# qhy991/llama.cpp-quant-gemm

Measured on NVIDIA B200. Metric: q4_0_q8_1_decode_gemv_hbm_gbs, higher is better.
Workload: dtype u4 x s8 -> s32 (dp4a), fp32 fold

## Files before the change

### llama.cpp-quant-gemm_b200/csrc/gemv.cu

```cuda
#include <cstdlib>

#include "ptx.cuh"
#include "qgemm_common.cuh"

namespace qgemm {

constexpr int kGemvWarps = 8;
constexpr int kGemvThreads = (kGemvWarps + 1) * 32;
constexpr int kGemvMaxStages = 8;
constexpr int kGemvInflightTarget = 56 * 1024;
constexpr int kGemvSlotsOff = 128;
constexpr int kGemvAbarOff = kGemvSlotsOff + 2 * kGemvWarps * 8 * 4;
constexpr int kGemvActOff = (kGemvAbarOff + 8 + 127) / 128 * 128;
static_assert(2 * kGemvMaxStages * 8 <= kGemvSlotsOff, "ring barriers overlap the slots");
static_assert(kGemvAbarOff % 8 == 0 && kGemvAbarOff + 8 <= kGemvActOff, "abar must not overlap the bulk-copy destination");
constexpr int kGemvSmemBudget = 110 * 1024;
constexpr int kGemvCtasPerSm = 2;
constexpr int kGemvMaxGroup = 8;
constexpr int kGemvTileTarget = 24 * 1024;

template <int WT> struct Pair { static constexpr int words = Fmt<WT>::bytes / 2; };

template <int WT>
__device__ __forceinline__ void load_pair(const uint8_t* p, uint32_t (&x)[Pair<WT>::words]) {
    if constexpr (WT == QGEMM_TYPE_Q5_1) {
        const uint4* q = reinterpret_cast<const uint4*>(p);
#pragma unroll
        for (int i = 0; i < 3; i++) {
            const uint4 v = q[i];
            x[4 * i] = v.x; x[4 * i + 1] = v.y; x[4 * i + 2] = v.z; x[4 * i + 3] = v.w;
        }
    } else if constexpr (WT == QGEMM_TYPE_Q4_1) {
        const uint2* q = reinterpret_cast<const uint2*>(p);
#pragma unroll
        for (int i = 0; i < 5; i++) {
            const uint2 v = q[i];
            x[2 * i] = v.x; x[2 * i + 1] = v.y;
        }
    } else {
        const uint32_t* q = reinterpret_cast<const uint32_t*>(p);
#pragma unroll
        for (int i = 0; i < Pair<WT>::words; i++) x[i] = q[i];
    }
}

__device__ __forceinline__ void expand4(const uint32_t (&q)[4], uint32_t (&w)[8]) {
#pragma unroll
    for (int i = 0; i < 4; i++) {
        w[i] = q[i] & 0x0f0f0f0fu;
        w[i + 4] = q[i] & 0xf0f0f0f0u;
    }
}
template <int WT>
__device__ __forceinline__ int pair_sumi(const uint32_t (&w)[8], const int (&a)[8]) {
    if constexpr (Fmt<WT>::bits == 4) {
        int lo = 0, hi = 0;
#pragma unroll
        for (int i = 0; i < 4; i++) {
            lo = dp4a_us(w[i], a[i], lo);
            hi = dp4a_us(w[i + 4], a[i + 4], hi);
        }
        return lo + (hi >> 4);
    } else {
        return block_sumi<WT>(w, a);
    }
}
__device__ __forceinline__ void expand5(const uint32_t (&q)[4], uint32_t qh, uint32_t (&w)[8]) {
#pragma unroll
    for (int i = 0; i < 4; i++) {
        w[i] = (q[i] & 0x0f0f0f0fu) | spread_qh4(qh, 4 * i);
        w[i + 4] = ((q[i] >> 4) & 0x0f0f0f0fu) | spread_qh4(qh, 16 + 4 * i);
    }
}

template <int WT>
__device__ __forceinline__ void expand_pair(const uint32_t (&x)[Pair<WT>::words], uint32_t (&w)[2][8], WScale (&ws)[2]) {
    auto fs = [](uint32_t lo, uint32_t hi) { return __funnelshift_r(lo, hi, 16); };
    if constexpr (WT == QGEMM_TYPE_Q4_0) {
        ws[0] = {half_bits_to_float(x[0]), 0.f};
        ws[1] = {half_bits_to_float(x[4] >> 16), 0.f};
        const uint32_t q0[4] = {fs(x[0], x[1]), fs(x[1], x[2]), fs(x[2], x[3]), fs(x[3], x[4])};
        const uint32_t q1[4] = {x[5], x[6], x[7], x[8]};
        expand4(q0, w[0]);
        expand4(q1, w[1]);
    } else if constexpr (WT == QGEMM_TYPE_Q4_1) {
        ws[0] = {half_bits_to_float(x[0]), half_bits_to_float(x[0] >> 16)};
        ws[1] = {half_bits_to_float(x[5]), half_bits_to_float(x[5] >> 16)};
        const uint32_t q0[4] = {x[1], x[2], x[3], x[4]};
        const uint32_t q1[4] = {x[6], x[7], x[8], x[9]};
        expand4(q0, w[0]);
        expand4(q1, w[1]);
    } else if constexpr (WT == QGEMM_TYPE_Q5_0) {
        ws[0] = {half_bits_to_float(x[0]), 0.f};
        ws[1] = {half_bits_to_float(x[5] >> 16), 0.f};
        const uint32_t q0[4] = {fs(x[1], x[2]), fs(x[2], x[3]), fs(x[3], x[4]), fs(x[4], x[5])};
        const uint32_t q1[4] = {x[7], x[8], x[9], x[10]};
        expand5(q0, fs(x[0], x[1]), w[0]);
        expand5(q1, x[6], w[1]);
    } else if constexpr (WT == QGEMM_TYPE_Q5_1) {
        ws[0] = {half_bits_to_float(x[0]), half_bits_to_float(x[0] >> 16)};
        ws[1] = {half_bits_to_float(x[6]), half_bits_to_float(x[6] >> 16)};
        const uint32_t q0[4] = {x[2], x[3], x[4], x[5]};
        const uint32_t q1[4] = {x[8], x[9], x[10], x[11]};
        expand5(q0, x[1], w[0]);
        expand5(q1, x[7], w[1]);
    } else {
        ws[0] = {half_bits_to_float(x[0]), 0.f};
        ws[1] = {half_bits_to_float(x[8] >> 16), 0.f};
#pragma unroll
        for (int i = 0; i < 8; i++) {
            w[0][i] = fs(x[i], x[i + 1]);
            w[1][i] = x[9 + i];
        }
    }
}

struct ActPair {
    int q[2][8];
    ActScale s[2];
};

struct GemvParams {
    const uint8_t* act;
    const uint8_t* wgt;
    float* C;
    int F, nb;
    int64_t ldc_t, ldc_f;
    int RT;
    int WPR;
    int stages;
    int stage_bytes;
    int pdl;
    int nocompute;
    int act_bulk;
    PeerOut peer;
    const uint8_t* pf_ptr;
    unsigned long long pf_bytes;
    int nmat;
    const uint8_t* wgt_m[kGemvMaxGroup];
    float* C_m[kGemvMaxGroup];
    int fstart[kGemvMaxGroup + 1];
    float skew;
#ifdef QGEMM_GEMV_TRACE
    int trace_slot;
#endif
};

#ifdef QGEMM_GEMV_TRACE
constexpr int kTraceSlots = 256, kTraceCtas = 304;
__device__ unsigned long long g_gemv_trace[kTraceSlots][kTraceCtas][6];
__device__ __forceinline__ unsigned long long gtimer() {
    unsigned long long t;
    asm volatile("mov.u64 %0, %%globaltimer;" : "=l"(t));
    return t;
}
#define GEMV_TRACE(i) do { if (threadIdx.x == 0 && blockIdx.x < kTraceCtas) g_gemv_trace[p.trace_slot][blockIdx.x][i] = gtimer(); } while (0)
#else
#define GEMV_TRACE(i)
#endif

struct TileRef { int m, local, rows; };
__device__ __forceinline__ TileRef tile_at(const GemvParams& p, int r0, int r_end) {
    TileRef t{0, r0, min(p.RT, r_end - r0)};
    if (p.nmat > 1) {
        int m = 0;
        while (m + 1 < p.nmat && r0 >= p.fstart[m + 1]) m++;
        t.m = m;
        t.local = r0 - p.fstart[m];
        t.rows = min(t.rows, p.fstart[m + 1] - r0);
    }
    return t;
}

template <int WT, int TT, int PPL, bool kMsExact, bool kFull>
__global__ void __launch_bounds__(kGemvThreads, kGemvCtasPerSm) gemv_kernel(const GemvParams p) {
    using Fm = Fmt<WT>;
    extern __shared__ __align__(128) uint8_t smem[];
    const int tid = threadIdx.x, warp = tid >> 5, lane = tid & 31;
    const int nb = p.nb, np = nb >> 1;

    uint64_t* full = reinterpret_cast<uint64_t*>(smem);
    uint64_t* empty = full + kGemvMaxStages;
    float* slots = reinterpret_cast<float*>(smem + kGemvSlotsOff);
    uint8_t* a_raw = smem + kGemvActOff;
    float4* a_scale = reinterpret_cast<float4*>(smem + kGemvActOff);
    uint4* a_qs = reinterpret_cast<uint4*>(smem + kGemvActOff + (size_t)TT * np * 16);
    const uint32_t act_bytes = (PPL > 0) ? (uint32_t)TT * nb * 36u : (uint32_t)TT * nb * 40u;
    uint8_t* stage0 = smem + (((uint32_t)kGemvActOff + act_bytes + 127u) & ~127u);

    auto span_at = [&](unsigned c) -> int {
        if (c >= gridDim.x) return p.F;
        const float x = (float)c / (float)gridDim.x;
        const float g = x * (1.0f + 0.5f * p.skew) - 0.5f * p.skew * x * x;
        return min(p.F, (int)((float)p.F * g + 0.5f));
    };
    const int r_begin = p.skew == 0.0f ? (int)(((int64_t)p.F * blockIdx.x) / gridDim.x) : span_at(blockIdx.x);
    const int r_end = p.skew == 0.0f ? (int)(((int64_t)p.F * (blockIdx.x + 1)) / gridDim.x) : span_at(blockIdx.x + 1);
    const size_t rowbytes = (size_t)nb * Fm::bytes;

    uint64_t* abar = reinterpret_cast<uint64_t*>(smem + kGemvAbarOff);
    if (tid == 0) {
        for (int s = 0; s < p.stages; s++) {
            ptx::mbar_init(&full[s], 1);
            ptx::mbar_init(&empty[s], kGemvWarps);
        }
        ptx::mbar_init(abar, 1);
        ptx::fence_mbar_init();
    }
    __syncthreads();
    if (p.pdl) ptx::griddep_launch_dependents();

    if (warp == kGemvWarps) {
        if (lane == 0) {
            int s = 0;
            uint32_t ph = 0;
            for (int r0 = r_begin; r0 < r_end;) {
                const TileRef tr = tile_at(p, r0, r_end);
                const uint8_t* src = (p.nmat > 1 ? p.wgt_m[tr.m] : p.wgt) + (size_t)tr.local * rowbytes;
                const uint32_t bytes = (uint32_t)(tr.rows * rowbytes);
                ptx::mbar_wait(&empty[s], ph ^ 1);
                ptx::mbar_arrive_expect_tx(&full[s], bytes);
                ptx::bulk_g2s(stage0 + (size_t)s * p.stage_bytes, src, bytes, &full[s]);
                if (++s == p.stages) { s = 0; ph ^= 1; }
                r0 += tr.rows;
            }
            if (p.pf_ptr) {
                const unsigned long long chunk = ((p.pf_bytes / gridDim.x) + 15ull) & ~15ull;
                unsigned long long off = chunk * blockIdx.x;
                const unsigned long long end = min(off + chunk, p.pf_bytes & ~15ull);
                for (; off < end; off += 16384ull)
                    ptx::bulk_prefetch_l2(p.pf_ptr + off, (uint32_t)min(16384ull, end - off));
            }
        }
        return;
    }

    GEMV_TRACE(0);
    if (p.pdl == 1) ptx::griddep_wait();
    GEMV_TRACE(1);
    if (p.peer.world > 1) {
        if (tid == 0) peer_wait_prior(p.peer);
        ptx::bar_sync(1, kGemvWarps * 32);
    }
    const int WPR = p.WPR;
    const int rpp = kGemvWarps / WPR;
    const int rslot = warp / WPR, sub = warp - rslot * WPR;

    ActPair areg[PPL > 0 ? TT : 1][PPL > 0 ? PPL : 1];
    if constexpr (PPL > 0) {
        const uint32_t* a32 = reinterpret_cast<const uint32_t*>(p.act);
        uint32_t* dst = reinterpret_cast<uint32_t*>(a_raw);
        const int total = TT * nb * 9;
        if (p.act_bulk) {
            if (tid == 0) {
                ptx::mbar_arrive_expect_tx(abar, (uint32_t)total * 4u);
                ptx::bulk_g2s(a_raw, p.act, (uint32_t)total * 4u, abar);
            }
            ptx::mbar_wait(abar, 0);
            GEMV_TRACE(4);
        } else {
            for (int i = tid; i < total; i += kGemvWarps * 32) dst[i] = __ldg(a32 + i);
            ptx::bar_sync(1, kGemvWarps * 32);
        }
#pragma unroll
        for (int j = 0; j < PPL; j++) {
            const int pg = (j * WPR + sub) * 32 + lane;
#pragma unroll
            for (int t = 0; t < TT; t++) {
                if (kFull || j < PPL - 1 || pg < np) {
                    const uint32_t* w = dst + ((size_t)t * nb + 2 * pg) * 9;
#pragma unroll
                    for (int b = 0; b < 2; b++) {
                        const uint32_t ds = w[9 * b];
                        areg[t][j].s[b] = prep_act_scale<WT, kMsExact>(half_bits_to_float(ds), half_bits_to_float(ds >> 16));
#pragma unroll
                        for (int i = 0; i < 8; i++) areg[t][j].q[b][i] = (int)w[9 * b + 1 + i];
                    }
                }
            }
        }
    } else {
        const uint32_t* a32 = reinterpret_cast<const uint32_t*>(p.act);
        float* sc = reinterpret_cast<float*>(a_scale);
        uint32_t* qs = reinterpret_cast<uint32_t*>(a_qs);
        const int total = TT * nb * 9;
        for (int i = tid; i < total; i += kGemvWarps * 32) {
            const int blk = i / 9, wd = i - blk * 9;
            const int t = blk / nb, b = blk - t * nb;
            const uint32_t v = __ldg(a32 + i);
            if (wd == 0) {
                const ActScale ps = prep_act_scale<WT, kMsExact>(half_bits_to_float(v), half_bits_to_float(v >> 16));
                float* d = sc + ((size_t)t * np + (b >> 1)) * 4 + (b & 1) * 2;
                d[0] = ps.d;
                d[1] = ps.s;
            } else {
                const int e = wd - 1;
                const int quad = (b & 1) * 2 + (e >> 2);
                qs[(((size_t)t * 4 + quad) * np + (b >> 1)) * 4 + (e & 3)] = v;
            }
        }
        ptx::bar_sync(1, kGemvWarps * 32);
    }

    GEMV_TRACE(2);
    int s = 0, spar = 0;
    uint32_t ph = 0;
    const int npl = (PPL > 0) ? PPL : (np + WPR * 32 - 1) / (WPR * 32);
    for (int g0 = r_begin; g0 < r_end;) {
        const TileRef tr = tile_at(p, g0, r_end);
        const int r0 = tr.local, rows = tr.rows;
        float* Cm = p.nmat > 1 ? p.C_m[tr.m] : p.C;
        g0 += rows;
        ptx::mbar_wait(&full[s], ph);
        const uint8_t* tile = stage0 + (size_t)s * p.stage_bytes;
        for (int pass = 0; pass * rpp < rows && !p.nocompute; pass++) {
            const int r = pass * rpp + rslot;
            float acc[TT];
#pragma unroll
            for (int tt = 0; tt < TT; tt++) acc[tt] = 0.f;
            if (r < rows) {
                const uint8_t* rowp = tile + (size_t)r * rowbytes;
                auto do_pair = [&](int j, int pg) {
                    uint32_t x[Pair<WT>::words];
                    uint32_t w[2][8];
                    WScale ws[2];
                    load_pair<WT>(rowp + (size_t)pg * (2 * Fm::bytes), x);
                    expand_pair<WT>(x, w, ws);
#pragma unroll
                    for (int tt = 0; tt < TT; tt++) {
                        if constexpr (PPL > 0) {
                            const ActPair& a = areg[tt][j];
                            acc[tt] = fold_block_pre<WT>(acc[tt], pair_sumi<WT>(w[0], a.q[0]), ws[0], a.s[0]);
                            acc[tt] = fold_block_pre<WT>(acc[tt], pair_sumi<WT>(w[1], a.q[1]), ws[1], a.s[1]);
                        } else {
                            const float4 sc = a_scale[(size_t)tt * np + pg];
                            int a0[8], a1[8];
                            const uint4 q0 = a_qs[((size_t)tt * 4 + 0) * np + pg];
                            const uint4 q1 = a_qs[((size_t)tt * 4 + 1) * np + pg];
                            const uint4 q2 = a_qs[((size_t)tt * 4 + 2) * np + pg];
                            const uint4 q3 = a_qs[((size_t)tt * 4 + 3) * np + pg];
                            a0[0] = q0.x; a0[1] = q0.y; a0[2] = q0.z; a0[3] = q0.w;
                            a0[4] = q1.x; a0[5] = q1.y; a0[6] = q1.z; a0[7] = q1.w;
                            a1[0] = q2.x; a1[1] = q2.y; a1[2] = q2.z; a1[3] = q2.w;
                            a1[4] = q3.x; a1[5] = q3.y; a1[6] = q3.z; a1[7] = q3.w;
                            acc[tt] = fold_block_pre<WT>(acc[tt], pair_sumi<WT>(w[0], a0), ws[0], ActScale{sc.x, sc.y});
                            acc[tt] = fold_block_pre<WT>(acc[tt], pair_sumi<WT>(w[1], a1), ws[1], ActScale{sc.z, sc.w});
                        }
                    }
                };
                if constexpr (PPL > 0) {
#pragma unroll
                    for (int j = 0; j < PPL; j++) {
                        const int pg = (j * WPR + sub) * 32 + lane;
                        if (kFull || j < PPL - 1 || pg < np) do_pair(j, pg);
                    }
                } else {
                    for (int j = 0; j < npl; j++) {
                        const int pg = (j * WPR + sub) * 32 + lane;
                        if (pg < np) do_pair(0, pg);
                    }
                }
            }
#pragma unroll
            for (int tt = 0; tt < TT; tt++) {
#pragma unroll
                for (int o = 16; o > 0; o >>= 1) acc[tt] += __shfl_xor_sync(0xffffffffu, acc[tt], o);
            }
            if (WPR == 1) {
                if (r < rows && lane < TT) {
                    float v = acc[0];
#pragma unroll
                    for (int tt = 1; tt < TT; tt++) v = (lane == tt) ? acc[tt] : v;
                    peer_store(p.peer, Cm, (int64_t)lane * p.ldc_t + (int64_t)(r0 + r) * p.ldc_f, v, tr.m);
                }
            } else {
                float* sl = slots + spar * (kGemvWarps * 8);
                if (lane == 0) {
#pragma unroll
                    for (int tt = 0; tt < TT; tt++) sl[warp * 8 + tt] = acc[tt];
                }
                ptx::bar_sync(2 + rslot, WPR * 32);
                if (sub == 0 && lane < TT && r < rows) {
                    float v = 0.f;
                    for (int k = 0; k < WPR; k++) v += sl[(rslot * WPR + k) * 8 + lane];
                    peer_store(p.peer, Cm, (int64_t)lane * p.ldc_t + (int64_t)(r0 + r) * p.ldc_f, v, tr.m);
                }
                spar ^= 1;
            }
        }
        __syncwarp();
        if (lane == 0) ptx::mbar_arrive(&empty[s]);
        if (++s == p.stages) { s = 0; ph ^= 1; }
    }
    GEMV_TRACE(3);
    if (p.peer.world > 1) {
        if (!(p.peer.dbg & 4)) __threadfence();
        ptx::bar_sync(1, kGemvWarps * 32);
        if (tid == 0) peer_signal_done(p.peer, gridDim.x);
    }
    if (p.pdl == 2) ptx::griddep_wait();
}

struct GemvPlan {
    int tt;
    int ppl;
    int wpr;
    int rt;
    int stages, stage_bytes;
    size_t smem;
};

static bool gemv_plan(int wtype, int T, int F, int K, int grid, bool pdl, GemvPlan* pl);

bool gemv_supported(int wtype, const void* act, const void* wgt, int F, int K) {
    const int nb = K / 32;
    const size_t rowbytes = (size_t)nb * block_bytes(wtype);
    if (F < 1 || nb < 2 || (nb & 1)) return false;
    if (rowbytes % 16 != 0 || rowbytes > 64 * 1024) return false;
    if (reinterpret_cast<uintptr_t>(wgt) % 16 != 0) return false;
    if (reinterpret_cast<uintptr_t>(act) % 4 != 0) return false;
    GemvPlan pl;
    return gemv_plan(wtype, 1, F, K, 1, false, &pl);
}

static bool gemv_plan(int wtype, int T, int F, int K, int grid, bool pdl, GemvPlan* pl) {
    const int nb = K / 32, np = nb / 2;
    const size_t rowbytes = (size_t)nb * block_bytes(wtype);
    for (int tt = min(T, 8); tt >= 1; tt--) {
        int ppl = 0, wpr = 1;
        for (int w = 1; w <= kGemvWarps; w <<= 1) {
            const int need = (np + 32 * w - 1) / (32 * w);
            if (need * tt <= 3) { ppl = need; wpr = w; break; }
        }
        if (QGEMM_ENV("QGEMM_GEMV_FORCE_SMEM")) ppl = 0;
        if (ppl == 0) {
            wpr = 1;
            while (wpr < kGemvWarps && np > 64 * wpr) wpr <<= 1;
        }
        const int rpp = kGemvWarps / wpr;
        int rt = rpp;
        while (rt < 8 && (size_t)(2 * rt) * rowbytes <= (size_t)kGemvTileTarget) rt <<= 1;
        if (const char* e = QGEMM_ENV("QGEMM_GEMV_RT")) rt = max(rpp, atoi(e) / rpp * rpp);
        const size_t fixed = kGemvActOff + (size_t)tt * nb * (ppl == 0 ? 40 : 36) + 128;
        auto stage_of = [&](int r) { return (int)(((size_t)r * rowbytes + 127) / 128 * 128); };
        while (rt > 1 && fixed + 2 * (size_t)stage_of(rt) > (size_t)kGemvSmemBudget) rt >>= 1;
        const int stage_bytes = stage_of(rt);
        if (fixed + 2 * (size_t)stage_bytes > (size_t)kGemvSmemBudget) continue;
        int stages = (int)(((size_t)kGemvSmemBudget - fixed) / stage_bytes);
        stages = max(2, min(kGemvMaxStages, stages));
        const int rows_per_cta = (F + grid - 1) / grid;
        stages = max(2, min(stages, (rows_per_cta + rt - 1) / rt));
        stages = max(2, min(stages, kGemvInflightTarget / stage_bytes));
        (void)pdl;
        if (const char* e = QGEMM_ENV("QGEMM_GEMV_STAGES")) stages = max(2, min(kGemvMaxStages, atoi(e)));
        *pl = {tt, ppl, wpr, rt, stages, stage_bytes, fixed + (size_t)stages * stage_bytes};
        return true;
    }
    return false;
}

template <int WT, int TT, int PPL>
static cudaError_t launch_gemv_inst(const GemvParams& p, size_t smem, int grid, bool ms_exact, cudaStream_t st) {
    auto launch = [&](auto kernel, int variant) -> cudaError_t {
        (void)variant;
        if (cudaError_t e = smem_optin(reinterpret_cast<const void*>(kernel), smem)) return e;
        cudaLaunchConfig_t cfg{};
        cfg.gridDim = dim3(grid);
        cfg.blockDim = dim3(kGemvThreads);
        cfg.dynamicSmemBytes = smem;
        cfg.stream = st;
        cudaLaunchAttribute at[1];
        at[0].id = cudaLaunchAttributeProgrammaticStreamSerialization;
        at[0].val.programmaticStreamSerializationAllowed = 1;
        cfg.attrs = at;
        cfg.numAttrs = p.pdl ? 1 : 0;
        return cudaLaunchKernelEx(&cfg, kernel, p);
    };
    cudaError_t e;
    const bool full = PPL > 0 && (p.nb / 2) == PPL * p.WPR * 32;
    if constexpr (Fmt<WT>::m >= 0) {
        if (full) e = ms_exact ? launch(gemv_kernel<WT, TT, PPL, true, true>, 2) : launch(gemv_kernel<WT, TT, PPL, false, true>, 3);
        else e = ms_exact ? launch(gemv_kernel<WT, TT, PPL, true, false>, 1) : launch(gemv_kernel<WT, TT, PPL, false, false>, 0);
    } else {
        e = full ? launch(gemv_kernel<WT, TT, PPL, false, true>, 3) : launch(gemv_kernel<WT, TT, PPL, false, false>, 0);
    }
    note_launch();
    return e;
}

template <int WT>
static cudaError_t launch_gemv_wt(const GemvPlan& pl, const GemvParams& p, int grid, bool ms, cudaStream_t st) {
#define QG_CASE(TTv, PPLv) \
    if (pl.tt == TTv && pl.ppl == PPLv) return launch_gemv_inst<WT, TTv, PPLv>(p, pl.smem, grid, ms, st);
    QG_CASE(1, 1) QG_CASE(1, 2) QG_CASE(1, 3) QG_CASE(2, 1) QG_CASE(3, 1)
    QG_CASE(1, 0) QG_CASE(2, 0) QG_CASE(3, 0) QG_CASE(4, 0) QG_CASE(5, 0) QG_CASE(6, 0) QG_CASE(7, 0) QG_CASE(8, 0)
#undef QG_CASE
    return cudaErrorInvalidValue;
}

struct GemvGroup { int nmat; const void* wgt[kGemvMaxGroup]; float* C[kGemvMaxGroup]; int F[kGemvMaxGroup]; };

cudaError_t launch_gemv(int wtype, const void* act, const void* wgt, float* C, int T, int F, int K, int64_t ldc_t,
                        int64_t ldc_f, uint32_t flags, int num_sms, cudaStream_t st, const PeerOut* peer,
                        const void* pf_ptr, size_t pf_bytes, const GemvGroup* group);

cudaError_t launch_gemv(int wtype, const void* act, const void* wgt, float* C, int T, int F, int K, int64_t ldc_t,
                        int64_t ldc_f, uint32_t flags, int num_sms, cudaStream_t st, const PeerOut* peer,
                        const void* pf_ptr, size_t pf_bytes) {
    return launch_gemv(wtype, act, wgt, C, T, F, K, ldc_t, ldc_f, flags, num_sms, st, peer, pf_ptr, pf_bytes, nullptr);
}

cudaError_t launch_gemv(int wtype, const void* act, const void* wgt, float* C, int T, int F, int K, int64_t ldc_t,
                        int64_t ldc_f, uint32_t flags, int num_sms, cudaStream_t st, const PeerOut* peer,
                        const void* pf_ptr, size_t pf_bytes, const GemvGroup* group) {
    const int nb = K / 32;
    const bool ms = flags & QGEMM_MS_EXACT;
    GemvPlan pl;
    int ctas_per_sm = kGemvCtasPerSm;
    if (const char* e = QGEMM_ENV("QGEMM_GEMV_CTAS")) ctas_per_sm = max(1, min(kGemvCtasPerSm, atoi(e)));
    const int grid = min(F, ctas_per_sm * num_sms);
    const bool pdl = flags & QGEMM_WEIGHTS_STATIC;
    if (!gemv_plan(wtype, T, F, K, grid, pdl, &pl)) return cudaErrorInvalidValue;
    for (int t0 = 0; t0 < T; t0 += pl.tt) {
        GemvPlan cur = pl;
        if (T - t0 < pl.tt && !gemv_plan(wtype, T - t0, F, K, grid, pdl, &cur)) return cudaErrorInvalidValue;
        GemvParams p;
        p.act = (const uint8_t*)act + (size_t)t0 * nb * kQ81Bytes;
        p.wgt = (const uint8_t*)wgt;
        p.C = C + (int64_t)t0 * ldc_t;
        p.F = F; p.nb = nb; p.ldc_t = ldc_t; p.ldc_f = ldc_f;
        p.RT = cur.rt; p.WPR = cur.wpr; p.stages = cur.stages; p.stage_bytes = cur.stage_bytes;
        p.pdl = pdl ? ((flags & QGEMM_INPUTS_READY) ? 2 : 1) : 0;
        p.nocompute = QGEMM_ENV("QGEMM_GEMV_NOCOMPUTE") ? 1 : 0;
        p.act_bulk = (reinterpret_cast<uintptr_t>(p.act) % 16 == 0 && ((size_t)cur.tt * nb * kQ81Bytes) % 16 == 0 &&
                      !QGEMM_ENV("QGEMM_GEMV_NO_ACT_BULK")) ? 1 : 0;
        p.pf_ptr = (t0 + pl.tt >= T && reinterpret_cast<uintptr_t>(pf_ptr) % 16 == 0) ? (const uint8_t*)pf_ptr : nullptr;
        p.pf_bytes = pf_bytes;
        p.skew = QGEMM_ENV("QGEMM_GEMV_SKEW") ? (float)atof(QGEMM_ENV("QGEMM_GEMV_SKEW")) : (F >= 8 * grid ? 0.28f : 0.0f);
#ifdef QGEMM_GEMV_TRACE
        {
            static int seq = 0;
            p.trace_slot = seq++ % kTraceSlots;
        }
#endif
        p.nmat = 0;
        if (group && group->nmat == 1) {
            p.wgt = (const uint8_t*)group->wgt[0];
            p.C = group->C[0] + (int64_t)t0 * ldc_t;
        } else if (group) {
            p.nmat = group->nmat;
            p.fstart[0] = 0;
            for (int m = 0; m < group->nmat; m++) {
                p.wgt_m[m] = (const uint8_t*)group->wgt[m];
                p.C_m[m] = group->C[m] + (int64_t)t0 * ldc_t;
                p.fstart[m + 1] = p.fstart[m] + group->F[m];
            }
        }
        p.peer = PeerOut{};
        if (peer) {
            if (T > pl.tt) return cudaErrorInvalidValue;
            p.peer = *peer;
        }
        cudaError_t e;
        switch (wtype) {
        case QGEMM_TYPE_Q4_0: e = launch_gemv_wt<QGEMM_TYPE_Q4_0>(cur, p, grid, ms, st); break;
        case QGEMM_TYPE_Q4_1: e = launch_gemv_wt<QGEMM_TYPE_Q4_1>(cur, p, grid, ms, st); break;
        case QGEMM_TYPE_Q5_0: e = launch_gemv_wt<QGEMM_TYPE_Q5_0>(cur, p, grid, ms, st); break;
        case QGEMM_TYPE_Q5_1: e = launch_gemv_wt<QGEMM_TYPE_Q5_1>(cur, p, grid, ms, st); break;
        case QGEMM_TYPE_Q8_0: e = launch_gemv_wt<QGEMM_TYPE_Q8_0>(cur, p, grid, ms, st); break;
        default: e = cudaErrorInvalidValue;
        }
        if (e != cudaSuccess) return e;
    }
    return cudaSuccess;
}


constexpr int kChainMaxSteps = 160;
constexpr int kChainMaxMat = 3;
constexpr int kChainQStride = 1536 * 36;

struct ChainStep {
    const uint8_t* act;
    const float* x;
    const float* gate;
    const uint8_t* wgt[kChainMaxMat];
    float* C[kChainMaxMat];
    int fstart[kChainMaxMat + 1];
    int nb;
    int ldc_f;
    unsigned char nmat, RT, WPR, ppl, full, wait;
};

template <int NS> struct ChainParams {
    int nsteps;
    int stages, stage_bytes;
    uint32_t act_bytes;
    unsigned* sync;
    uint8_t* qscratch;
    int pdl;
    const uint8_t* pf_ptr;
    unsigned long long pf_bytes;
    ChainStep st[NS];
};
constexpr int kChainSmall = 8;

__device__ __forceinline__ uint32_t ld_acquire_gpu(const unsigned* p) {
    uint32_t v;
    asm volatile("ld.acquire.gpu.global.u32 %0, [%1];" : "=r"(v) : "l"(p) : "memory");
    return v;
}

struct ChainTile { int m, local, rows; };
__device__ __forceinline__ ChainTile chain_tile_at(const ChainStep& st, int r0, int r_end) {
    int m = 0;
    while (m + 1 < st.nmat && r0 >= st.fstart[m + 1]) m++;
    return {m, r0 - st.fstart[m], min(min((int)st.RT, r_end - r0), st.fstart[m + 1] - r0)};
}

__device__ __forceinline__ int chain_round_half_away(float v) {
    const float t = truncf(v);
    const float r = v - t;
    int q = __float2int_rz(t);
    if (fabsf(r) >= 0.5f) q += (v < 0.0f) ? -1 : 1;
    return q;
}
__device__ __noinline__ void chain_quantize_block_lanes(const float* x, const float* gate, uint8_t* out, int lane) {
    float v = __ldcg(x + lane);
    if (gate) v = __fmul_rn(__fdiv_rn(v, __fadd_rn(1.0f, expf(-v))), __ldcg(gate + lane));
    float amax = fabsf(v);
#pragma unroll
    for (int o = 16; o > 0; o >>= 1) amax = fmaxf(amax, __shfl_xor_sync(0xffffffffu, amax, o));
    float sum = 0.0f;
#pragma unroll
    for (int j = 0; j < 32; j++) sum = __fadd_rn(sum, __shfl_sync(0xffffffffu, v, j));
    const float d = __fdiv_rn(amax, 127.0f);
    const float id = (d > 0.0f) ? __fdiv_rn(1.0f, d) : 0.0f;
    const int q = max(-128, min(127, chain_round_half_away(__fmul_rn(v, id))));
    out[4 + lane] = (uint8_t)(q & 0xff);
    if (lane == 0)
        *reinterpret_cast<uint32_t*>(out) =
            (uint32_t)__half_as_ushort(__float2half_rn(d)) | ((uint32_t)__half_as_ushort(__float2half_rn(sum)) << 16);
}

template <int WT, int PPL, bool kFull>
__device__ __forceinline__ void chain_consume(const ChainStep& st, const int r_begin, const int r_end, const uint32_t* araw,
                                              const uint8_t* stage0, const int stage_bytes, const int nstages, uint64_t* full,
                                              uint64_t* empty, float* slots, int& s, uint32_t& ph, int& spar) {
    using Fm = Fmt<WT>;
    const int tid = threadIdx.x, warp = tid >> 5, lane = tid & 31;
    const int nb = st.nb, np = nb >> 1;
    const int WPR = st.WPR;
    const int rpp = kGemvWarps / WPR;
    const int rslot = warp / WPR, sub = warp - rslot * WPR;
    const size_t rowbytes = (size_t)nb * Fm::bytes;

    ActPair areg[PPL];
#pragma unroll
    for (int j = 0; j < PPL; j++) {
        const int pg = (j * WPR + sub) * 32 + lane;
        if (kFull || j < PPL - 1 || pg < np) {
            const uint32_t* w = araw + (size_t)(2 * pg) * 9;
#pragma unroll
            for (int b = 0; b < 2; b++) {
                const uint32_t ds = w[9 * b];
                areg[j].s[b] = prep_act_scale<WT, false>(half_bits_to_float(ds), half_bits_to_float(ds >> 16));
#pragma unroll
                for (int i = 0; i < 8; i++) areg[j].q[b][i] = (int)w[9 * b + 1 + i];
            }
        }
    }
    for (int g0 = r_begin; g0 < r_end;) {
        const ChainTile tr = chain_tile_at(st, g0, r_end);
        const int r0 = tr.local, rows = tr.rows;
        float* Cm = st.C[tr.m];
        g0 += rows;
        ptx::mbar_wait(&full[s], ph);
        const uint8_t* tile = stage0 + (size_t)s * stage_bytes;
        for (int pass = 0; pass * rpp < rows; pass++) {
            const int r = pass * rpp + rslot;
            float acc = 0.f;
            if (r < rows) {
                const uint8_t* rowp = tile + (size_t)r * rowbytes;
#pragma unroll
                for (int j = 0; j < PPL; j++) {
                    const int pg = (j * WPR + sub) * 32 + lane;
                    if (kFull || j < PPL - 1 || pg < np) {
                        uint32_t x[Pair<WT>::words];
                        uint32_t w[2][8];
                        WScale ws[2];
                        load_pair<WT>(rowp + (size_t)pg * (2 * Fm::bytes), x);
                        expand_pair<WT>(x, w, ws);
                        acc = fold_block_pre<WT>(acc, pair_sumi<WT>(w[0], areg[j].q[0]), ws[0], areg[j].s[0]);
                        acc = fold_block_pre<WT>(acc, pair_sumi<WT>(w[1], areg[j].q[1]), ws[1], areg[j].s[1]);
                    }
                }
            }
#pragma unroll
            for (int o = 16; o > 0; o >>= 1) acc += __shfl_xor_sync(0xffffffffu, acc, o);
            if (WPR == 1) {
                if (r < rows && lane == 0) Cm[(int64_t)(r0 + r) * st.ldc_f] = acc;
            } else {
                float* sl = slots + spar * (kGemvWarps * 8);
                if (lane == 0) sl[warp * 8] = acc;
                ptx::bar_sync(2 + rslot, WPR * 32);
                if (sub == 0 && lane == 0 && r < rows) {
                    float v = 0.f;
                    for (int k = 0; k < WPR; k++) v += sl[(rslot * WPR + k) * 8];
                    Cm[(int64_t)(r0 + r) * st.ldc_f] = v;
                }
                spar ^= 1;
            }
        }
        __syncwarp();
        if (lane == 0) ptx::mbar_arrive(&empty[s]);
        if (++s == nstages) { s = 0; ph ^= 1; }
    }
}

template <int WT, int NS>
__global__ void __launch_bounds__(kGemvThreads, kGemvCtasPerSm) gemv_chain_kernel(const __grid_constant__ ChainParams<NS> p) {
    using Fm = Fmt<WT>;
    extern __shared__ __align__(128) uint8_t smem[];
    const int tid = threadIdx.x, warp = tid >> 5, lane = tid & 31;
    uint64_t* full = reinterpret_cast<uint64_t*>(smem);
    uint64_t* empty = full + kGemvMaxStages;
    float* slots = reinterpret_cast<float*>(smem + kGemvSlotsOff);
    uint64_t* abar = reinterpret_cast<uint64_t*>(smem + kGemvAbarOff);
    uint8_t* a_raw = smem + kGemvActOff;
    uint8_t* stage0 = smem + (((uint32_t)kGemvActOff + p.act_bytes + 127u) & ~127u);
    const unsigned grid = gridDim.x;

    if (tid == 0) {
        for (int s = 0; s < p.stages; s++) {
            ptx::mbar_init(&full[s], 1);
            ptx::mbar_init(&empty[s], kGemvWarps);
        }
        ptx::mbar_init(abar, 1);
        ptx::fence_mbar_init();
    }
    __syncthreads();
    if (p.pdl) ptx::griddep_launch_dependents();

    if (warp == kGemvWarps) {
        if (lane == 0) {
            int s = 0;
            uint32_t ph = 0;
            for (int k = 0; k < p.nsteps; k++) {
                const ChainStep& st = p.st[k];
                const int F = st.fstart[st.nmat];
                const int r_begin = (int)(((int64_t)F * blockIdx.x) / grid);
                const int r_end = (int)(((int64_t)F * (blockIdx.x + 1)) / grid);
                const size_t rowbytes = (size_t)st.nb * Fm::bytes;
                for (int r0 = r_begin; r0 < r_end;) {
                    const ChainTile tr = chain_tile_at(st, r0, r_end);
                    const uint8_t* src = st.wgt[tr.m] + (size_t)tr.local * rowbytes;
                    const uint32_t bytes = (uint32_t)(tr.rows * rowbytes);
                    ptx::mbar_wait(&empty[s], ph ^ 1);
                    ptx::mbar_arrive_expect_tx(&full[s], bytes);
                    ptx::bulk_g2s(stage0 + (size_t)s * p.stage_bytes, src, bytes, &full[s]);
                    if (++s == p.stages) { s = 0; ph ^= 1; }
                    r0 += tr.rows;
                }
            }
            if (p.pf_ptr) {
                const unsigned long long chunk = ((p.pf_bytes / grid) + 15ull) & ~15ull;
                unsigned long long off = chunk * blockIdx.x;
                const unsigned long long end = min(off + chunk, p.pf_bytes & ~15ull);
                for (; off < end; off += 16384ull)
                    ptx::bulk_prefetch_l2(p.pf_ptr + off, (uint32_t)min(16384ull, end - off));
            }
        }
        return;
    }

    if (p.pdl) ptx::griddep_wait();
    int s = 0, spar = 0;
    uint32_t ph = 0, aph = 0;
    for (int k = 0; k < p.nsteps; k++) {
        const ChainStep& st = p.st[k];
        const int F = st.fstart[st.nmat];
        const int r_begin = (int)(((int64_t)F * blockIdx.x) / grid);
        const int r_end = (int)(((int64_t)F * (blockIdx.x + 1)) / grid);
        if (st.act) {
            if (tid == 0) {
                if (st.wait && k > 0)
                    while (ld_acquire_gpu(p.sync + (k - 1)) < grid) __nanosleep(20);
                const uint32_t bytes = (uint32_t)st.nb * 36u;
                ptx::mbar_arrive_expect_tx(abar, bytes);
                ptx::bulk_g2s(a_raw, st.act, bytes, abar);
            }
            ptx::mbar_wait(abar, aph);
            aph ^= 1;
        } else {
            if (k > 0) {
                if (tid == 0)
                    while (ld_acquire_gpu(p.sync + (k - 1)) < grid) __nanosleep(20);
                ptx::bar_sync(1, kGemvWarps * 32);
            }
            uint8_t* qbuf = p.qscratch + (size_t)(k & 1) * kChainQStride;
            for (int b = (int)blockIdx.x + warp * (int)grid; b < st.nb; b += kGemvWarps * (int)grid)
                chain_quantize_block_lanes(st.x + (size_t)b * 32, st.gate ? st.gate + (size_t)b * 32 : nullptr, qbuf + (size_t)b * 36, lane);
            __threadfence();
            ptx::bar_sync(1, kGemvWarps * 32);
            if (tid == 0) {
                atomicAdd(p.sync + p.nsteps + 1 + k, 1u);
                while (ld_acquire_gpu(p.sync + p.nsteps + 1 + k) < grid) __nanosleep(20);
            }
            ptx::bar_sync(1, kGemvWarps * 32);
            const uint32_t* src = reinterpret_cast<const uint32_t*>(qbuf);
            uint32_t* dst = reinterpret_cast<uint32_t*>(a_raw);
            for (int i = tid; i < st.nb * 9; i += kGemvWarps * 32) dst[i] = __ldcg(src + i);
            ptx::fence_proxy_async();
            ptx::bar_sync(1, kGemvWarps * 32);
        }
        const uint32_t* araw = reinterpret_cast<const uint32_t*>(a_raw);
#define QG_CHAIN_CASE(P, FULL) \
    chain_consume<WT, P, FULL>(st, r_begin, r_end, araw, stage0, p.stage_bytes, p.stages, full, empty, slots, s, ph, spar)
        if (st.full) {
            if (st.ppl == 1) QG_CHAIN_CASE(1, true);
            else if (st.ppl == 2) QG_CHAIN_CASE(2, true);
            else QG_CHAIN_CASE(3, true);
        } else {
            if (st.ppl == 1) QG_CHAIN_CASE(1, false);
            else if (st.ppl == 2) QG_CHAIN_CASE(2, false);
            else QG_CHAIN_CASE(3, false);
        }
#undef QG_CHAIN_CASE
        if (lane == 0) __threadfence();
        ptx::bar_sync(1, kGemvWarps * 32);
        if (tid == 0) atomicAdd(p.sync + k, 1u);
    }
    if (tid == 0) {
        if (atomicAdd(p.sync + p.nsteps, 1u) == grid - 1) {
            for (int k = 0; k <= 2 * p.nsteps; k++) p.sync[k] = 0u;
        }
    }
}

struct ChainStepHost {
    const void* act; const float* x; const float* gate;
    int nmat; const void* wgt[kChainMaxMat]; float* C[kChainMaxMat]; int F[kChainMaxMat];
    int K; int ldc_f; int wait;
};

int gemv_chain_max_steps() { return kChainMaxSteps; }
static size_t gemv_chain_counter_bytes(int) { return ((size_t)(2 * kChainMaxSteps + 1) * sizeof(unsigned) + 255) / 256 * 256; }
size_t gemv_chain_sync_bytes(int nsteps) { return gemv_chain_counter_bytes(nsteps) + 2 * (size_t)kChainQStride; }

template <int NS>
static bool gemv_chain_plan(int wtype, const ChainStepHost* steps, int nsteps, int grid, ChainParams<NS>* out, size_t* smem) {
    if (nsteps < 1 || nsteps > NS) return false;
    int stage_bytes = 0;
    size_t act_bytes = 0;
    for (int k = 0; k < nsteps; k++) {
        const ChainStepHost& h = steps[k];
        if (h.nmat < 1 || h.nmat > kChainMaxMat) return false;
        const int nb = h.K / 32;
        int Ftot = 0;
        for (int m = 0; m < h.nmat; m++) {
            if (!gemv_supported(wtype, h.act ? h.act : (const void*)h.x, h.wgt[m], h.F[m], h.K)) return false;
            Ftot += h.F[m];
        }
        if (h.act) {
            if (reinterpret_cast<uintptr_t>(h.act) % 16 != 0 || ((size_t)nb * kQ81Bytes) % 16 != 0) return false;
        } else {
            if (reinterpret_cast<uintptr_t>(h.x) % 16 != 0 || (h.gate && reinterpret_cast<uintptr_t>(h.gate) % 16 != 0)) return false;
        }
        GemvPlan pl;
        if (!gemv_plan(wtype, 1, Ftot, h.K, grid, true, &pl) || pl.tt != 1 || pl.ppl < 1 || pl.ppl > 3) return false;
        ChainStep& st = out->st[k];
        st = ChainStep{};
        st.act = (const uint8_t*)h.act; st.x = h.x; st.gate = h.gate;
        st.fstart[0] = 0;
        for (int m = 0; m < h.nmat; m++) {
            st.wgt[m] = (const uint8_t*)h.wgt[m];
            st.C[m] = h.C[m];
            st.fstart[m + 1] = st.fstart[m] + h.F[m];
        }
        for (int m = h.nmat; m < kChainMaxMat; m++) st.fstart[m + 1] = st.fstart[h.nmat];
        st.nb = nb; st.ldc_f = h.ldc_f;
        st.nmat = (unsigned char)h.nmat; st.RT = (unsigned char)pl.rt; st.WPR = (unsigned char)pl.wpr; st.ppl = (unsigned char)pl.ppl;
        st.full = (nb / 2) == pl.ppl * pl.wpr * 32 ? 1 : 0;
        st.wait = h.wait ? 1 : 0;
        stage_bytes = max(stage_bytes, (int)(((size_t)pl.rt * nb * block_bytes(wtype) + 127) / 128 * 128));
        act_bytes = max(act_bytes, (size_t)nb * kQ81Bytes);
    }
    const size_t fixed = (((size_t)kGemvActOff + act_bytes + 127) & ~(size_t)127);
    if (fixed + 2 * (size_t)stage_bytes > (size_t)kGemvSmemBudget) return false;
    int stages = (int)(((size_t)kGemvSmemBudget - fixed) / stage_bytes);
    stages = max(2, min(kGemvMaxStages, stages));
    if (const char* e = QGEMM_ENV("QGEMM_CHAIN_STAGES")) stages = max(2, min(stages, atoi(e)));
    out->nsteps = nsteps;
    out->stages = stages;
    out->stage_bytes = stage_bytes;
    out->act_bytes = (uint32_t)act_bytes;
    *smem = fixed + (size_t)stages * stage_bytes;
    return true;
}

template <int WT, int NS>
static cudaError_t launch_chain_wt(const ChainParams<NS>& p, size_t smem, int num_sms, cudaStream_t st) {
    auto kernel = gemv_chain_kernel<WT, NS>;
    if (cudaError_t e = smem_optin(reinterpret_cast<const void*>(kernel), smem)) return e;
    int occ = 0;
    if (cudaError_t e = cudaOccupancyMaxActiveBlocksPerMultiprocessor(&occ, kernel, kGemvThreads, smem)) return e;
    if (occ < kGemvCtasPerSm) return cudaErrorLaunchOutOfResources;
    cudaLaunchConfig_t cfg{};
    cfg.gridDim = dim3(kGemvCtasPerSm * num_sms);
    cfg.blockDim = dim3(kGemvThreads);
    cfg.dynamicSmemBytes = smem;
    cfg.stream = st;
    cudaLaunchAttribute at[1];
    at[0].id = cudaLaunchAttributeProgrammaticStreamSerialization;
    at[0].val.programmaticStreamSerializationAllowed = 1;
    cfg.attrs = at;
    cfg.numAttrs = p.pdl ? 1 : 0;
    cudaError_t e = cudaLaunchKernelEx(&cfg, kernel, p);
    note_launch();
    return e;
}

template <int NS>
static cudaError_t launch_chain_ns(int wtype, const ChainStepHost* steps, int nsteps, uint32_t flags, unsigned* sync, int num_sms,
                                   cudaStream_t st, const void* pf_ptr, size_t pf_bytes) {
    static thread_local ChainParams<NS> p;
    size_t smem = 0;
    const int grid = kGemvCtasPerSm * num_sms;
    if (!gemv_chain_plan<NS>(wtype, steps, nsteps, grid, &p, &smem)) return cudaErrorNotSupported;
    p.sync = sync;
    p.qscratch = reinterpret_cast<uint8_t*>(sync) + gemv_chain_counter_bytes(nsteps);
    p.pdl = (flags & QGEMM_WEIGHTS_STATIC) ? 1 : 0;
    p.pf_ptr = reinterpret_cast<uintptr_t>(pf_ptr) % 16 == 0 ? (const uint8_t*)pf_ptr : nullptr;
    p.pf_bytes = pf_bytes;
    switch (wtype) {
    case QGEMM_TYPE_Q4_0: return launch_chain_wt<QGEMM_TYPE_Q4_0, NS>(p, smem, num_sms, st);
    case QGEMM_TYPE_Q4_1: return launch_chain_wt<QGEMM_TYPE_Q4_1, NS>(p, smem, num_sms, st);
    case QGEMM_TYPE_Q5_0: return launch_chain_wt<QGEMM_TYPE_Q5_0, NS>(p, smem, num_sms, st);
    case QGEMM_TYPE_Q5_1: return launch_chain_wt<QGEMM_TYPE_Q5_1, NS>(p, smem, num_sms, st);
    case QGEMM_TYPE_Q8_0: return launch_chain_wt<QGEMM_TYPE_Q8_0, NS>(p, smem, num_sms, st);
    default: return cudaErrorInvalidValue;
    }
}

cudaError_t launch_gemv_chain(int wtype, const ChainStepHost* steps, int nsteps, uint32_t flags, unsigned* sync, int num_sms,
                              cudaStream_t st, const void* pf_ptr, size_t pf_bytes) {
    if ((flags & QGEMM_MS_EXACT) && (wtype == QGEMM_TYPE_Q4_1 || wtype == QGEMM_TYPE_Q5_1)) return cudaErrorNotSupported;
    const int grid = kGemvCtasPerSm * num_sms;
    for (int k = 0; k < nsteps; k++) {
        int Ftot = 0;
        for (int m = 0; m < steps[k].nmat && m < kChainMaxMat; m++) Ftot += steps[k].F[m];
        if (Ftot < grid) return cudaErrorNotSupported;
    }
    if (nsteps <= kChainSmall) return launch_chain_ns<kChainSmall>(wtype, steps, nsteps, flags, sync, num_sms, st, pf_ptr, pf_bytes);
    return launch_chain_ns<kChainMaxSteps>(wtype, steps, nsteps, flags, sync, num_sms, st, pf_ptr, pf_bytes);
}

}

#ifdef QGEMM_GEMV_TRACE
extern "C" __attribute__((visibility("default"))) int qgemm_debug_read_gemv_trace(unsigned long long* dst, size_t bytes) {
    return (int)cudaMemcpyFromSymbol(dst, qgemm::g_gemv_trace, bytes < sizeof(qgemm::g_gemv_trace) ? bytes : sizeof(qgemm::g_gemv_trace));
}
#endif
```

Measured before the change: 4239.

## Process two rows per warp and split warps into groups over alternating stages

For single-token Q4_0/Q4_1 decode with few pairs per lane, each warp now computes two rows at once, loading both rows' weight pairs before expanding them so more loads are in flight per lane. When WPR allows, the eight consumer warps split into two groups that take alternating pipeline stages, and the empty-barrier count drops to match the group size. Each warp also releases its stage early, right after its last loads, so the producer can refill sooner. The risks are higher register pressure, subtle correctness issues in the early release and odd-row handling, and a direct store path that bypasses peer_store when world is 1.

```diff
diff --git a/llama.cpp-quant-gemm_b200/csrc/gemv.cu b/llama.cpp-quant-gemm_b200/csrc/gemv.cu
--- a/llama.cpp-quant-gemm_b200/csrc/gemv.cu
+++ b/llama.cpp-quant-gemm_b200/csrc/gemv.cu
@@ -159,6 +159,10 @@
 #define GEMV_TRACE(i)
 #endif
 
+__device__ constexpr int gemv_rows_per_warp(int wt, int tt, int ppl) {
+    return (tt == 1 && ppl > 0 && ppl <= 2 && (wt == QGEMM_TYPE_Q4_0 || wt == QGEMM_TYPE_Q4_1)) ? 2 : 1;
+}
+
 struct TileRef { int m, local, rows; };
 __device__ __forceinline__ TileRef tile_at(const GemvParams& p, int r0, int r_end) {
     TileRef t{0, r0, min(p.RT, r_end - r0)};
@@ -198,11 +202,14 @@
     const int r_end = p.skew == 0.0f ? (int)(((int64_t)p.F * (blockIdx.x + 1)) / gridDim.x) : span_at(blockIdx.x + 1);
     const size_t rowbytes = (size_t)nb * Fm::bytes;
 
+    constexpr bool kTwoRows = gemv_rows_per_warp(WT, TT, PPL) == 2;
+    const int gw = (kTwoRows && p.WPR <= kGemvWarps / 2) ? kGemvWarps / 2 : kGemvWarps;
+
     uint64_t* abar = reinterpret_cast<uint64_t*>(smem + kGemvAbarOff);
     if (tid == 0) {
         for (int s = 0; s < p.stages; s++) {
             ptx::mbar_init(&full[s], 1);
-            ptx::mbar_init(&empty[s], kGemvWarps);
+            ptx::mbar_init(&empty[s], gw);
         }
         ptx::mbar_init(abar, 1);
         ptx::fence_mbar_init();
@@ -305,92 +312,163 @@
     GEMV_TRACE(2);
     int s = 0, spar = 0;
     uint32_t ph = 0;
-    const int npl = (PPL > 0) ? PPL : (np + WPR * 32 - 1) / (WPR * 32);
-    for (int g0 = r_begin; g0 < r_end;) {
-        const TileRef tr = tile_at(p, g0, r_end);
-        const int r0 = tr.local, rows = tr.rows;
-        float* Cm = p.nmat > 1 ? p.C_m[tr.m] : p.C;
-        g0 += rows;
-        ptx::mbar_wait(&full[s], ph);
-        const uint8_t* tile = stage0 + (size_t)s * p.stage_bytes;
-        for (int pass = 0; pass * rpp < rows && !p.nocompute; pass++) {
-            const int r = pass * rpp + rslot;
-            float acc[TT];
-#pragma unroll
-            for (int tt = 0; tt < TT; tt++) acc[tt] = 0.f;
-            if (r < rows) {
-                const uint8_t* rowp = tile + (size_t)r * rowbytes;
-                auto do_pair = [&](int j, int pg) {
-                    uint32_t x[Pair<WT>::words];
-                    uint32_t w[2][8];
-                    WScale ws[2];
-                    load_pair<WT>(rowp + (size_t)pg * (2 * Fm::bytes), x);
-                    expand_pair<WT>(x, w, ws);
-#pragma unroll
-                    for (int tt = 0; tt < TT; tt++) {
-                        if constexpr (PPL > 0) {
-                            const ActPair& a = areg[tt][j];
-                            acc[tt] = fold_block_pre<WT>(acc[tt], pair_sumi<WT>(w[0], a.q[0]), ws[0], a.s[0]);
-                            acc[tt] = fold_block_pre<WT>(acc[tt], pair_sumi<WT>(w[1], a.q[1]), ws[1], a.s[1]);
-                        } else {
-                            const float4 sc = a_scale[(size_t)tt * np + pg];
-                            int a0[8], a1[8];
-                            const uint4 q0 = a_qs[((size_t)tt * 4 + 0) * np + pg];
-                            const uint4 q1 = a_qs[((size_t)tt * 4 + 1) * np + pg];
-                            const uint4 q2 = a_qs[((size_t)tt * 4 + 2) * np + pg];
-                            const uint4 q3 = a_qs[((size_t)tt * 4 + 3) * np + pg];
-                            a0[0] = q0.x; a0[1] = q0.y; a0[2] = q0.z; a0[3] = q0.w;
-                            a0[4] = q1.x; a0[5] = q1.y; a0[6] = q1.z; a0[7] = q1.w;
-                            a1[0] = q2.x; a1[1] = q2.y; a1[2] = q2.z; a1[3] = q2.w;
-                            a1[4] = q3.x; a1[5] = q3.y; a1[6] = q3.z; a1[7] = q3.w;
-                            acc[tt] = fold_block_pre<WT>(acc[tt], pair_sumi<WT>(w[0], a0), ws[0], ActScale{sc.x, sc.y});
-                            acc[tt] = fold_block_pre<WT>(acc[tt], pair_sumi<WT>(w[1], a1), ws[1], ActScale{sc.z, sc.w});
+    if constexpr (kTwoRows) {
+        const int ngroups = kGemvWarps / gw, g = warp / gw;
+        const int gs = gw / WPR, gslot = (warp - g * gw) / WPR;
+        const int rpt = 2 * gs;
+        const int half = lane >> 4;
+        for (int g0 = r_begin, k = 0; g0 < r_end; k++) {
+            const TileRef tr = tile_at(p, g0, r_end);
+            g0 += tr.rows;
+            if (k % ngroups != g) {
+                if (++s == p.stages) { s = 0; ph ^= 1; }
+                continue;
+            }
+            float* Cm = p.nmat > 1 ? p.C_m[tr.m] : p.C;
+            ptx::mbar_wait(&full[s], ph);
+            const uint8_t* tile = stage0 + (size_t)s * p.stage_bytes;
+            const int npass = p.nocompute ? 0 : (tr.rows + rpt - 1) / rpt;
+            if (npass == 0) {
+                __syncwarp();
+                if (lane == 0) ptx::mbar_arrive(&empty[s]);
+            }
+            for (int pass = 0; pass < npass; pass++) {
+                const int r = pass * rpt + gslot;
+                const uint8_t* rowp[2] = {tile + (size_t)r * rowbytes, tile + (size_t)(r + gs < tr.rows ? r + gs : r) * rowbytes};
+                float acc[2] = {0.f, 0.f};
+#pragma unroll
+                for (int j = 0; j < PPL; j++) {
+                    const int pg = (j * WPR + sub) * 32 + lane;
+                    const bool on = r < tr.rows && (kFull || j < PPL - 1 || pg < np);
+                    uint32_t x[2][Pair<WT>::words];
+                    if (on) {
+#pragma unroll
+                        for (int i = 0; i < 2; i++) load_pair<WT>(rowp[i] + (size_t)pg * (2 * Fm::bytes), x[i]);
+                    }
+                    if (j == PPL - 1 && pass == npass - 1) {
+                        __syncwarp();
+                        if (lane == 0) ptx::mbar_arrive(&empty[s]);
+                    }
+                    if (on) {
+#pragma unroll
+                        for (int i = 0; i < 2; i++) {
+                            uint32_t w[2][8];
+                            WScale ws[2];
+                            expand_pair<WT>(x[i], w, ws);
+                            const ActPair& a = areg[0][j];
+                            acc[i] = fold_block_pre<WT>(acc[i], pair_sumi<WT>(w[0], a.q[0]), ws[0], a.s[0]);
+                            acc[i] = fold_block_pre<WT>(acc[i], pair_sumi<WT>(w[1], a.q[1]), ws[1], a.s[1]);
                         }
                     }
-                };
-                if constexpr (PPL > 0) {
-#pragma unroll
-                    for (int j = 0; j < PPL; j++) {
-                        const int pg = (j * WPR + sub) * 32 + lane;
-                        if (kFull || j < PPL - 1 || pg < np) do_pair(j, pg);
+                }
+                float v = (half ? acc[1] : acc[0]) + __shfl_xor_sync(0xffffffffu, half ? acc[0] : acc[1], 16);
+#pragma unroll
+                for (int o = 8; o > 0; o >>= 1) v += __shfl_xor_sync(0xffffffffu, v, o);
+                const int row = r + half * gs;
+                if (WPR > 1) {
+                    float* sl = slots + spar * (kGemvWarps * 8);
+                    if ((lane & 15) == 0) sl[warp * 8 + half] = v;
+                    ptx::bar_sync(2 + rslot, WPR * 32);
+                    v = 0.f;
+                    for (int q = 0; q < WPR; q++) v += sl[(rslot * WPR + q) * 8 + half];
+                    spar ^= 1;
+                }
+                if ((lane & 15) == 0 && sub == 0 && row < tr.rows) {
+                    const int64_t idx = (int64_t)(tr.local + row) * p.ldc_f;
+                    if (p.peer.world > 1) peer_store(p.peer, Cm, idx, v, tr.m);
+                    else Cm[idx] = v;
+                }
+            }
+            if (++s == p.stages) { s = 0; ph ^= 1; }
+        }
+    } else {
+        const int npl = (PPL > 0) ? PPL : (np + WPR * 32 - 1) / (WPR * 32);
+        for (int g0 = r_begin; g0 < r_end;) {
+            const TileRef tr = tile_at(p, g0, r_end);
+            const int r0 = tr.local, rows = tr.rows;
+            float* Cm = p.nmat > 1 ? p.C_m[tr.m] : p.C;
+            g0 += rows;
+            ptx::mbar_wait(&full[s], ph);
+            const uint8_t* tile = stage0 + (size_t)s * p.stage_bytes;
+            for (int pass = 0; pass * rpp < rows && !p.nocompute; pass++) {
+                const int r = pass * rpp + rslot;
+                float acc[TT];
+    #pragma unroll
+                for (int tt = 0; tt < TT; tt++) acc[tt] = 0.f;
+                if (r < rows) {
+                    const uint8_t* rowp = tile + (size_t)r * rowbytes;
+                    auto do_pair = [&](int j, int pg) {
+                        uint32_t x[Pair<WT>::words];
+                        uint32_t w[2][8];
+                        WScale ws[2];
+                        load_pair<WT>(rowp + (size_t)pg * (2 * Fm::bytes), x);
+                        expand_pair<WT>(x, w, ws);
+    #pragma unroll
+                        for (int tt = 0; tt < TT; tt++) {
+                            if constexpr (PPL > 0) {
+                                const ActPair& a = areg[tt][j];
+                                acc[tt] = fold_block_pre<WT>(acc[tt], pair_sumi<WT>(w[0], a.q[0]), ws[0], a.s[0]);
+                                acc[tt] = fold_block_pre<WT>(acc[tt], pair_sumi<WT>(w[1], a.q[1]), ws[1], a.s[1]);
+                            } else {
+                                const float4 sc = a_scale[(size_t)tt * np + pg];
+                                int a0[8], a1[8];
+                                const uint4 q0 = a_qs[((size_t)tt * 4 + 0) * np + pg];
+                                const uint4 q1 = a_qs[((size_t)tt * 4 + 1) * np + pg];
+                                const uint4 q2 = a_qs[((size_t)tt * 4 + 2) * np + pg];
+                                const uint4 q3 = a_qs[((size_t)tt * 4 + 3) * np + pg];
+                                a0[0] = q0.x; a0[1] = q0.y; a0[2] = q0.z; a0[3] = q0.w;
+                                a0[4] = q1.x; a0[5] = q1.y; a0[6] = q1.z; a0[7] = q1.w;
+                                a1[0] = q2.x; a1[1] = q2.y; a1[2] = q2.z; a1[3] = q2.w;
+                                a1[4] = q3.x; a1[5] = q3.y; a1[6] = q3.z; a1[7] = q3.w;
+                                acc[tt] = fold_block_pre<WT>(acc[tt], pair_sumi<WT>(w[0], a0), ws[0], ActScale{sc.x, sc.y});
+                                acc[tt] = fold_block_pre<WT>(acc[tt], pair_sumi<WT>(w[1], a1), ws[1], ActScale{sc.z, sc.w});
+                            }
+                        }
+                    };
+                    if constexpr (PPL > 0) {
+    #pragma unroll
+                        for (int j = 0; j < PPL; j++) {
+                            const int pg = (j * WPR + sub) * 32 + lane;
+                            if (kFull || j < PPL - 1 || pg < np) do_pair(j, pg);
+                        }
+                    } else {
+                        for (int j = 0; j < npl; j++) {
+                            const int pg = (j * WPR + sub) * 32 + lane;
+                            if (pg < np) do_pair(0, pg);
+                        }
+                    }
+                }
+    #pragma unroll
+                for (int tt = 0; tt < TT; tt++) {
+    #pragma unroll
+                    for (int o = 16; o > 0; o >>= 1) acc[tt] += __shfl_xor_sync(0xffffffffu, acc[tt], o);
+                }
+                if (WPR == 1) {
+                    if (r < rows && lane < TT) {
+                        float v = acc[0];
+    #pragma unroll
+                        for (int tt = 1; tt < TT; tt++) v = (lane == tt) ? acc[tt] : v;
+                        peer_store(p.peer, Cm, (int64_t)lane * p.ldc_t + (int64_t)(r0 + r) * p.ldc_f, v, tr.m);
                     }
                 } else {
-                    for (int j = 0; j < npl; j++) {
-                        const int pg = (j * WPR + sub) * 32 + lane;
-                        if (pg < np) do_pair(0, pg);
+                    float* sl = slots + spar * (kGemvWarps * 8);
+                    if (lane == 0) {
+    #pragma unroll
+                        for (int tt = 0; tt < TT; tt++) sl[warp * 8 + tt] = acc[tt];
                     }
+                    ptx::bar_sync(2 + rslot, WPR * 32);
+                    if (sub == 0 && lane < TT && r < rows) {
+                        float v = 0.f;
+                        for (int k = 0; k < WPR; k++) v += sl[(rslot * WPR + k) * 8 + lane];
+                        peer_store(p.peer, Cm, (int64_t)lane * p.ldc_t + (int64_t)(r0 + r) * p.ldc_f, v, tr.m);
+                    }
+                    spar ^= 1;
                 }
             }
-#pragma unroll
-            for (int tt = 0; tt < TT; tt++) {
-#pragma unroll
-                for (int o = 16; o > 0; o >>= 1) acc[tt] += __shfl_xor_sync(0xffffffffu, acc[tt], o);
-            }
-            if (WPR == 1) {
-                if (r < rows && lane < TT) {
-                    float v = acc[0];
-#pragma unroll
-                    for (int tt = 1; tt < TT; tt++) v = (lane == tt) ? acc[tt] : v;
-                    peer_store(p.peer, Cm, (int64_t)lane * p.ldc_t + (int64_t)(r0 + r) * p.ldc_f, v, tr.m);
-                }
-            } else {
-                float* sl = slots + spar * (kGemvWarps * 8);
-                if (lane == 0) {
-#pragma unroll
-                    for (int tt = 0; tt < TT; tt++) sl[warp * 8 + tt] = acc[tt];
-                }
-                ptx::bar_sync(2 + rslot, WPR * 32);
-                if (sub == 0 && lane < TT && r < rows) {
-                    float v = 0.f;
-                    for (int k = 0; k < WPR; k++) v += sl[(rslot * WPR + k) * 8 + lane];
-                    peer_store(p.peer, Cm, (int64_t)lane * p.ldc_t + (int64_t)(r0 + r) * p.ldc_f, v, tr.m);
-                }
-                spar ^= 1;
-            }
-        }
-        __syncwarp();
-        if (lane == 0) ptx::mbar_arrive(&empty[s]);
-        if (++s == p.stages) { s = 0; ph ^= 1; }
+            __syncwarp();
+            if (lane == 0) ptx::mbar_arrive(&empty[s]);
+            if (++s == p.stages) { s = 0; ph ^= 1; }
+        }
     }
     GEMV_TRACE(3);
     if (p.peer.world > 1) {
```

New measurement: 4026, median of 6. 0.95x the previous value.
